# chalharu/rust-compression

Measured on AMD Instinct MI355X. Metric: BZip2 level-9 encode MB/s (input bytes, HBM-resident in and out: the kernels' rate; value_end_to_end is host buffer to host buffer at the C ABI), higher is better.
Workload: dtype u8/u32

## Files before the change

### rust-compression_amd/csrc/k_bwt.hip

```cpp
#include "bzgpu.h"
#include <algorithm>
#include <atomic>
#include <cstdio>
#include <cstdlib>
#include <vector>

namespace bzgpu {
constexpr u32 kGhSpan = 8;
constexpr u32 kSymSpan = 8;

enum { SRC_TEXT = 0, SRC_PAIRS = 1, SRC_MM = 2, SRC_WALK = 3, SRC_SURV = 4, SRC_LISTG = 5,
       SRC_TEXTK = 6, SRC_WALKK = 7, SRC_MMK = 8,
       SRC_MMC = 9,
       SRC_PERJ = 10,
       SRC_PACKED = 11,
       SRC_PERJK = 12 };
template <int SRC> struct src_is_list {
    static constexpr bool value = (SRC == SRC_PAIRS || SRC == SRC_SURV || SRC == SRC_LISTG || SRC == SRC_PERJ || SRC == SRC_PERJK || SRC == SRC_PACKED);
};

struct KeyInfo {
    u8 bits;
    u8 chars;
    u8 pad[2];
};

__device__ __forceinline__ u32 pkey(const u8 *__restrict__ pt, u32 j, u32 bits, u32 chars)
{
    const u32 bitpos = j * bits, kb = bits * chars;
    u64 v;
    __builtin_memcpy(&v, pt + (bitpos >> 3), 8);
    v = __builtin_bswap64(v);
    return (u32)(v >> (64u - (bitpos & 7u) - kb)) & (u32)((1ull << kb) - 1ull);
}

__device__ __forceinline__ u64 newbits_lane_word(const u64 *__restrict__ bits, size_t base, u32 wbase, u32 cnt, u32 l, bool fill)
{
    const u32 rowbase = wbase + l * 64u;
    u64 m = 0;
    if (l < 17u && rowbase < cnt) m = bits[(base + rowbase) >> 6];
    if (fill && l < 17u) {
        if (rowbase >= cnt) m = ~0ull;
        else if (cnt - rowbase < 64u) m |= ~0ull << (cnt - rowbase);
    }
    return m;
}

constexpr u32 kPerWords = kSlot / 64u;
constexpr u32 kPerSetBytes = 2u * kPerWords * 8u + ((kPerWords + 1u) * 4u + 7u) / 8u * 8u;
static_assert((size_t)kPerK * kPerSetBytes <= (size_t)kTilesPerBlock * 3 * kMaxBins * 4, "the period tables do not fit the digit-count slot");
__host__ __device__ __forceinline__ bool per_in_counts(const BwtArgs &a) { return a.gh_tiles != nullptr; }
__host__ __device__ __forceinline__ u32 per_kmax(const BwtArgs &a) { return per_in_counts(a) ? kPerK : (kSlot / kPerSetBytes < kPerK ? kSlot / kPerSetBytes : kPerK); }
__device__ __forceinline__ const u8 *per_set(const BwtArgs &a, u32 lb, u32 i)
{
    const u8 *base = per_in_counts(a) ? reinterpret_cast<const u8 *>(a.gh_tiles + (size_t)lb * kTilesPerBlock * 3 * kMaxBins)
                                      : a.flags + (size_t)lb * kSlot;
    return base + (size_t)i * kPerSetBytes;
}
__device__ __forceinline__ const u64 *per_mis(const BwtArgs &a, u32 lb, u32 i) { return reinterpret_cast<const u64 *>(per_set(a, lb, i)); }
__device__ __forceinline__ const u64 *per_lt(const BwtArgs &a, u32 lb, u32 i) { return per_mis(a, lb, i) + kPerWords; }
__device__ __forceinline__ const u32 *per_nxt(const BwtArgs &a, u32 lb, u32 i) { return reinterpret_cast<const u32 *>(per_mis(a, lb, i) + 2u * kPerWords); }
__device__ __forceinline__ u32 per_first_mis(const BwtArgs &a, u32 lb, u32 i, u32 x)
{
    const u32 w = x >> 6;
    const u64 here = per_mis(a, lb, i)[w] & (~0ull << (x & 63u));
    return here ? (w << 6) + (u32)__builtin_ctzll(here) : per_nxt(a, lb, i)[w + 1u];
}
__device__ __forceinline__ bool per_lt_at(const BwtArgs &a, u32 lb, u32 i, u32 n, u32 m)
{
    if (m >= n) m -= n;
    return (per_lt(a, lb, i)[m >> 6] >> (m & 63u)) & 1ull;
}
__device__ __forceinline__ bool per_key_ascending(const BwtArgs &a, u32 lb, u32 n, u32 depth, u32 j)
{
    const u32 kmax = per_kmax(a);
    for (u32 i = 0; i < kmax; ++i) {
        const u32 p = a.lin_p[(size_t)lb * kPerK + i];
        if (p == 0u) break;
        if (j + p < n) {
            const u32 m = per_first_mis(a, lb, i, j);
            if (m - j >= depth) return per_lt_at(a, lb, i, n, m);
        }
        if (j >= p) {
            const u32 m = per_first_mis(a, lb, i, j - p);
            if (m - (j - p) >= depth) return per_lt_at(a, lb, i, n, m);
        }
    }
    return true;
}

__device__ __forceinline__ bool per_ekey(const BwtArgs &a, u32 lb, const u8 *__restrict__ text, u32 n, u32 depth, u32 x, u32 &key)
{
    const u32 kmax = per_kmax(a);
    for (u32 i = 0; i < kmax; ++i) {
        const u32 p = a.lin_p[(size_t)lb * kPerK + i];
        if (p == 0u) break;
        if (p > depth) continue;
        const u32 m = per_first_mis(a, lb, i, x);
        const u32 e = m - x + p;
        if (e < depth) continue;
        u32 mp = (m >= n ? m - n : m) + p;
        mp = mp >= n ? mp - n : mp;
        const bool up = per_lt_at(a, lb, i, n, m);
        const u32 ec = e < 0xFFFFFu ? e : 0xFFFFFu;
        key = up ? ((1u << 28) | ((0xFFFFFu - ec) << 8) | (u32)text[mp]) : ((ec << 8) | (u32)text[mp]);
        return true;
    }
    return false;
}

constexpr u32 kLinkMax = 8;
__device__ __forceinline__ u8 *group_bytes(const BwtArgs &a, u32 lb)
{
    return a.per_aux + (size_t)lb * kMtfStride * 2u;
}

// ... 913 lines not shown
    const u32 gshift = 20u + kbits;
    const bool haveB = posB < len;
    u64 eA[16], eB[16];
    loc_fill(eA, s_e, posA, len, l, le_mask, gshift, gcarryA);
    if (haveB) loc_fill(eB, s_e, posB, len, l, le_mask, gshift, gcarryB);
    const u32 gbits = groups > 1u ? 32u - (u32)__builtin_clz(groups - 1u) : 0u;
    const u32 npass = (kbits + gbits + kLocBits - 1u) / kLocBits;
    u32 *cntA = s_cnt[w], *cntB = s_cnt[kLocWaves + w];
    u16 *cnt16 = reinterpret_cast<u16 *>(&s_cnt[0][0]);
#pragma unroll 1
    for (u32 p = 0; p < npass; ++p) {
        const u32 shift = 20u + p * kLocBits;
        u32 rnkA[16], rnkB[16];
        loc_rank(eA, rnkA, cntA, posA, len, l, shift);
        if (haveB) loc_rank(eB, rnkB, cntB, posB, len, l, shift);
        else {
#pragma unroll
            for (u32 q = 0; q < kLocBins / 2 / 64; ++q) cntB[q * 64u + l] = 0;
        }
        __syncthreads();
        u32 tot;
        {
            const u32 dg = threadIdx.x;
            u32 run = 0;
#pragma unroll
            for (u32 k = 0; k < kLocSets; ++k) {
                const u32 c = cnt16[k * kLocBins + dg];
                cnt16[k * kLocBins + dg] = (u16)run;
                run += c;
            }
            tot = run;
        }
        const u32 inc = wave_incl_sum(tot);
        if (l == 63) s_wsum[w] = inc;
        __syncthreads();
        {
            u32 carry = 0;
            for (u32 k = 0; k < w; ++k) carry += s_wsum[k];
            s_tpre[threadIdx.x] = (u16)(carry + inc - tot);
        }
        __syncthreads();
        loc_move(eA, rnkA, cntA, s_tpre, s_e, posA, len, l, shift);
        if (haveB) loc_move(eB, rnkB, cntB, s_tpre, s_e, posB, len, l, shift);
        __syncthreads();
        if (p + 1 < npass) {
            loc_reload(eA, s_e, posA, len, l);
            if (haveB) loc_reload(eB, s_e, posB, len, l);
        }
    }
    {
        bool bad = false;
        for (u32 i = threadIdx.x; i < len; i += kLocThreads) {
            const u64 x = s_e[i];
            if (i && (s_e[i - 1] >> 20) > (x >> 20)) bad = true;
            const u32 v = (u32)x & 0xFFFFFu;
            Vout[base + s0 + i] = v;
            Kout[base + s0 + i] = Rb[v] & ~kFinalBit;
        }
        if (__ballot(bad) && l == 0) s_bad = 1u;
    }
    __syncthreads();
    if (threadIdx.x == 0 && s_bad) atomicAdd(&a.loc_stats[LOC_STAT_SURV_FAIL], 1u);
}

template <bool INIT>
__global__ __launch_bounds__(kSortThreads) void k_group_flags(BwtArgs a, u32 step, const u32 *__restrict__ K,
                                                               const u32 *__restrict__ V,
                                                               const u8 *__restrict__ impure = nullptr)
{
    __shared__ int s_old, s_new;
    u32 tile, lb;
    xcd_remap(gridDim.x, a.nb, tile, lb);
    if (lb == 0xFFFFFFFFu) return;
    const BlockDesc d = a.blocks[lb];
    const u32 n = d.n;
    const u32 cnt = a.count[lb];
    const u32 start = tile * kSortTile;
    if (start >= cnt) return;
    const KeyInfo ki = reinterpret_cast<const KeyInfo *>(a.keyinfo)[lb];
    const u32 hm = INIT ? (u32)ki.chars % n : (((u32)ki.chars * 2u) << step) % n;
    const u8 *text = a.rle + d.rle_off;
    const u8 *pt = a.ptext + (size_t)lb * kSlot;
    const size_t base = (size_t)lb * kSlot;
    if (INIT && a.pb_gate[lb] == 0u) K = a.KA;
    if (threadIdx.x == 0) {
        s_old = -1;
        s_new = -1;
    }
    __syncthreads();
    const u32 w = threadIdx.x >> 6, l = threadIdx.x & 63u;
    int last_old = -1, last_new = -1;
    const u32 first = start + w * 1024u + l;
    u32 g[16], s1[16], s2[16];
    u32 pg0 = 0, ps10 = 0, ps20 = 0;
    {
        u32 jj[16];
#pragma unroll
        for (u32 r = 0; r < 16; ++r) {
            const u32 idx = first + r * 64u;
            const u32 c = idx < cnt ? idx : cnt - 1u;
            const u32 kk = ld_stream(K + base + c);
            const u32 t = ld_stream(V + base + c) + hm;
            jj[r] = t >= n ? t - n : t;
            g[r] = INIT ? 0u : kk;
            s1[r] = kk;
            s2[r] = 0;
        }
        u32 pj = 0;
        const bool need_prev = (l == 0) && (first > 0) && (first < cnt);
        if (need_prev) {
            const u32 kk = K[base + first - 1];
            pg0 = INIT ? 0u : kk;
            ps10 = kk;
            const u32 t = V[base + first - 1] + hm;
            pj = t >= n ? t - n : t;
        }
        if (INIT) {
#pragma unroll
            for (u32 r = 0; r < 16; ++r) s2[r] = pkey(pt, jj[r], ki.bits, ki.chars);
            if (need_prev) ps20 = pkey(pt, pj, ki.bits, ki.chars);
        } else if (impure) {
            const bool per = a.lin_p[(size_t)lb * kPerK] != 0u;
            const u64 d64 = ((u64)ki.chars * 2u) << step;
            const u32 depth = d64 < n ? (u32)d64 : n;
#pragma unroll
            for (u32 r = 0; r < 16; ++r) {
                const u32 jr = jj[r] >= hm ? jj[r] - hm : jj[r] + n - hm;
                const u32 im = impure[base + g[r]];
                u32 ek;
                s1[r] = (im == 2u || (per && im == 0u)) ? jr + 1u : ((per && a.per_wide && per_ekey(a, lb, text, n, depth, jr, ek)) ? ek + 1u : 0u);
            }
            if (need_prev) {
                const u32 jr = pj >= hm ? pj - hm : pj + n - hm;
                const u32 im = impure[base + pg0];
                u32 ek;
                ps10 = (im == 2u || (per && im == 0u)) ? jr + 1u : ((per && a.per_wide && per_ekey(a, lb, text, n, depth, jr, ek)) ? ek + 1u : 0u);
            }
        } else {
#pragma unroll
            for (u32 r = 0; r < 16; ++r) s1[r] = a.R[base + jj[r]];
            if (need_prev) ps10 = a.R[base + pj];
        }
    }
#pragma unroll
    for (u32 r = 0; r < 16; ++r) {
        const u32 idx = first + r * 64u;
        const bool ok = idx < cnt;
        u32 pg = wave_shr1(g[r]), p1 = wave_shr1(s1[r]), p2 = wave_shr1(s2[r]);
        const u32 qg = (r == 0) ? pg0 : wave_lane(g[(r + 15) & 15], 63);
        const u32 q1 = (r == 0) ? ps10 : wave_lane(s1[(r + 15) & 15], 63);
        const u32 q2 = (r == 0) ? ps20 : wave_lane(s2[(r + 15) & 15], 63);
        if (l == 0) {
            pg = qg;
            p1 = q1;
            p2 = q2;
        }
        bool ns = false;
        if (ok) {
            const bool os = (idx == 0) || (g[r] != pg);
            ns = os || (s1[r] != p1) || (s2[r] != p2);
            a.flags[base + idx] = (u8)((os ? 1u : 0u) | (ns ? 2u : 0u));
            if (os) last_old = (int)idx;
            if (ns) last_new = (int)idx;
        }
        const u64 mrow = __ballot(ns);
        if (l == 0 && idx < cnt) a.newbits[(base + idx) >> 6] = mrow;
    }
// ... 166 lines not shown
        const u32 mine = c0 + c1;
        const u32 inc = wave_incl_sum(mine);
        if (l == 63) s_wsum[w] = inc;
        u32 g0 = 0, g1 = 0;
        u32 *cur = a.bin_cursor + (size_t)lb * 1024u;
        if (c0) g0 = atomicAdd(&cur[b0], c0);
        if (c1) g1 = atomicAdd(&cur[b0 + 1], c1);
        __syncthreads();
        u32 carry = 0;
        for (u32 k = 0; k < w; ++k) carry += s_wsum[k];
        const u32 ex = carry + inc - mine;
        s_bpre[b0] = (u16)ex;
        s_bpre[b0 + 1] = (u16)(ex + c0);
        s_bcnt[b0] = (b0 << kRankBinShift) + g0;
        s_bcnt[b0 + 1] = ((b0 + 1u) << kRankBinShift) + g1;
    }
    __syncthreads();
#pragma unroll
    for (u32 r = 0; r < 16; ++r) {
        if (lrank[r] != 0xFFFFFFFFu) {
            const u32 bin = jv[r] >> kRankBinShift;
            const u32 pos = (u32)s_bpre[bin] + lrank[r];
            s_stage[pos] = word[r];
            s_binof[pos] = (u16)bin;
        }
    }
    __syncthreads();
    const u32 total = (cnt - start) < kSortTile ? (cnt - start) : kSortTile;
#pragma unroll
    for (u32 k = 0; k < 16; ++k) {
        const u32 i = k * kSortThreads + threadIdx.x;
        if (i < total) {
            const u32 bin = s_binof[i];
            W[base + s_bcnt[bin] + (i - (u32)s_bpre[bin])] = s_stage[i];
        }
    }
}

constexpr u32 kLbNone = 0xFFFFFu;
#ifdef BZ_REFINE_TIMING
#define RF_T(k) do { __syncthreads(); const u64 t_ = __builtin_readcyclecounter(); if (threadIdx.x == 0) atomicAdd(&a.loc_stats[16 + (INIT ? 8 : 0) + (k)], (u32)((t_ - t_prev) >> 4)); t_prev = t_; } while (0)
#else
#define RF_T(k) do { } while (0)
#endif
template <bool INIT>
__global__ __launch_bounds__(kSortThreads, 4) void k_group_refine(BwtArgs a, u32 step, u32 next_step, u32 round,
                                                                const u32 *__restrict__ K,
                                                                const u32 *__restrict__ V, u32 *__restrict__ W,
                                                                u32 epoch)
{
    constexpr u32 NW = kSortThreads / 64;
    __shared__ int s_carry_old, s_carry_new;
    __shared__ int s_wold[NW], s_wnew[NW];
    __shared__ u32 s_nonfinal, s_ticket;
    __shared__ u32 s_stage[kSortTile];
    __shared__ u16 s_binof[kSortTile];
    __shared__ u16 s_bpre[1024];
    __shared__ u16 s_bdst[1024];
    __shared__ u32 s_wsum[NW];
    u32 (*s_gh)[1024] = reinterpret_cast<u32 (*)[1024]>(s_stage);
    u32 *s_bcnt = s_stage + 2048;
#ifdef BZ_REFINE_TIMING
    u64 t_prev = __builtin_readcyclecounter();
#endif
    const u32 xcd = (u32)__builtin_amdgcn_s_getreg(20 | (3 << 11)) & 7u;
    const u32 my_tiles = a.tiles * ((a.nb + 7u - xcd) / 8u);
    if (threadIdx.x == 0) s_ticket = atomicAdd(&a.tickets[(size_t)epoch * 8u + xcd], 1u);
    __syncthreads();
    const u32 slot = s_ticket;
    if (slot >= my_tiles) return;
    const u32 b8 = slot / a.tiles;
    const u32 tile = slot - b8 * a.tiles;
    const u32 lb = b8 * 8u + xcd;
    const BlockDesc d = a.blocks[lb];
    const u32 n = d.n;
    const u8 *__restrict__ text = a.rle + d.rle_off;
    const u32 cnt = a.count[lb];
    const u32 start = tile * kSortTile;
    if (start >= cnt) return;
    const KeyInfo ki = reinterpret_cast<const KeyInfo *>(a.keyinfo)[lb];
    const u32 hm = INIT ? (u32)ki.chars % n : (((u32)ki.chars * 2u) << step) % n;
    const u8 *pt = a.ptext + (size_t)lb * kSlot;
    const size_t base = (size_t)lb * kSlot;
    if (INIT && a.pb_gate[lb] == 0u) K = a.KA;
    for (u32 i = threadIdx.x; i < 3072u; i += kSortThreads) s_stage[i] = 0;
    if (threadIdx.x == 0) s_nonfinal = 0;
    const u32 w = threadIdx.x >> 6, l = threadIdx.x & 63u;
    const u32 wbase = start + w * 1024u;
    const u32 first = wbase + l;

    RF_T(0);
    u32 gk[16], jv[16], s1[16], s2[16];
    u32 pg0 = 0, ps10 = 0, ps20 = 0;
    u32 ng0 = 0, ns10 = 0, ns20 = 0;
    const bool need_prev = (l == 0) && (first > 0) && (first < cnt);
    const bool need_next = (l == 63) && (wbase + 1024u < cnt);
    {
#pragma unroll
        for (u32 r = 0; r < 16; ++r) {
            const u32 idx = first + r * 64u;
            const u32 c = idx < cnt ? idx : cnt - 1u;
            const u32 kk = ld_stream(K + base + c);
            const u32 vv = ld_stream(V + base + c);
            if (INIT) {
                jv[r] = vv;
                const u32 t = vv + hm;
                s2[r] = t >= n ? t - n : t;
                gk[r] = 0u;
                s1[r] = kk;
            } else {
                jv[r] = vv & 0xFFFFFu;
                gk[r] = kk & 0xFFFFFu;
                s1[r] = (kk >> 20) | ((vv >> 20) << 12);
                s2[r] = 0u;
            }
        }
        u32 pj = 0, nj = 0;
        if (need_prev) {
            const u32 kk = K[base + wbase - 1], vv = V[base + wbase - 1];
            pg0 = INIT ? 0u : (kk & 0xFFFFFu);
            ps10 = INIT ? kk : ((kk >> 20) | ((vv >> 20) << 12));
            const u32 t = vv + hm;
            pj = t >= n ? t - n : t;
        }
        if (need_next) {
            const u32 kk = K[base + wbase + 1024u], vv = V[base + wbase + 1024u];
            ng0 = INIT ? 0u : (kk & 0xFFFFFu);
            ns10 = INIT ? kk : ((kk >> 20) | ((vv >> 20) << 12));
            const u32 t = vv + hm;
            nj = t >= n ? t - n : t;
        }
        if (INIT) {
#pragma unroll
            for (u32 r = 0; r < 16; ++r) s2[r] = pkey(pt, s2[r], ki.bits, ki.chars);
            if (need_prev) ps20 = pkey(pt, pj, ki.bits, ki.chars);
            if (need_next) ns20 = pkey(pt, nj, ki.bits, ki.chars);
        }
    }
    RF_T(1);
    u64 mo[16] = {}, mn[16];
    int wl_old = -1, wl_new = -1;
#pragma unroll
    for (u32 r = 0; r < 16; ++r) {
        const u32 idx = first + r * 64u;
        const bool ok = idx < cnt;
        u32 pg = wave_shr1(gk[r]), p1 = wave_shr1(s1[r]), p2 = wave_shr1(s2[r]);
        const u32 qg = (r == 0) ? pg0 : wave_lane(gk[(r + 15) & 15], 63);
        const u32 q1 = (r == 0) ? ps10 : wave_lane(s1[(r + 15) & 15], 63);
        const u32 q2 = (r == 0) ? ps20 : wave_lane(s2[(r + 15) & 15], 63);
        if (l == 0) {
            pg = qg;
            p1 = q1;
            p2 = q2;
        }
        const bool os = ok && ((idx == 0) || (!INIT && gk[r] != pg));
        const bool ns = ok && (os || (s1[r] != p1) || (s2[r] != p2));
        mn[r] = __ballot(ns);
        if (l == 0 && ok) a.newbits[(base + idx) >> 6] = mn[r];
        if (mn[r]) wl_new = (int)(wbase + r * 64u + 63u - __clzll(mn[r]));
        if (!INIT) {
            mo[r] = __ballot(os);
            if (mo[r]) wl_old = (int)(wbase + r * 64u + 63u - __clzll(mo[r]));
        }
    }
    bool next_after = true;
    if (need_next) next_after = (gk[15] != ng0) || (s1[15] != ns10) || (s2[15] != ns20);
    next_after = wave_lane((u32)next_after, 63) != 0u;
    if (l == 0) {
        s_wold[w] = INIT ? 0 : wl_old;
        s_wnew[w] = wl_new;
    }
    u32 finbits = 0;
    u32 lcol[16];
#pragma unroll
    for (u32 r = 0; r < 16; ++r) {
        const u32 idx = first + r * 64u;
        bool next_new;
        if (idx + 1 >= cnt) next_new = true;
        else if (l < 63) next_new = (mn[r] >> (l + 1)) & 1ull;
        else if (r < 15) next_new = mn[(r + 1) & 15] & 1ull;
        else next_new = next_after;
        const bool fin = (idx < cnt) && ((mn[r] >> l) & 1ull) && next_new;
        finbits |= (fin ? 1u : 0u) << r;
        lcol[r] = 0;
        if (INIT && fin) lcol[r] = text[jv[r] ? jv[r] - 1u : n - 1u];
    }
    __syncthreads();
    RF_T(2);
    if (threadIdx.x == 0) {
        int lo = INIT ? 0 : -1, ln = -1;
        for (u32 k = 0; k < NW; ++k) {
            lo = s_wold[k] > lo ? s_wold[k] : lo;
            ln = s_wnew[k] > ln ? s_wnew[k] : ln;
        }
        u32 *mystate = a.tile_state + ((size_t)lb * kTilesPerBlock + tile) * kMaxBins;
        const u32 etag = epoch << 22;
        const u32 f0 = etag | (tile ? kLbAgg : kLbIncl);
        const u32 vo = lo >= 0 ? (u32)lo : kLbNone, vn = ln >= 0 ? (u32)ln : kLbNone;
        st_sc1_x4(mystate, make_uint4(f0 | vo, f0 | vn, f0, f0));
        int co = -1, cn = -1;
        if (tile) {
            u32 spins = 0;
            for (u32 p = tile; p > 0 && (co < 0 || cn < 0);) {
                --p;
                const u32 *src = a.tile_state + ((size_t)lb * kTilesPerBlock + p) * kMaxBins;
                uint4 v = ld_sc1_x4(src);
                while ((v.x >> 22) != epoch || (v.x & kLbFlagMask) == 0u || (v.y >> 22) != epoch || (v.y & kLbFlagMask) == 0u) {
                    if (lb_give_up(spins, a.sort_err, kLbSpinMax >> 3)) {
                        atomicExch(a.sort_err, 1u);
                        v = make_uint4(etag | kLbIncl, etag | kLbIncl, 0, 0);
                        break;
                    }
                    __builtin_amdgcn_s_sleep(2);
                    v = ld_sc1_x4(src);
                }
                const u32 xo = v.x & kLbValMask, xn = v.y & kLbValMask;
                if (co < 0 && xo != kLbNone) co = (int)xo;
                if (cn < 0 && xn != kLbNone) cn = (int)xn;
            }
// ... 1167 lines not shown
        bytes[i] = 0;
        seconds[i] = 0;
    }
}

template <int SRC, int BITS>
static void radix_pass(hipStream_t st, const BwtArgs &a, u32 shift, u32 h, const u32 *Kin, const u32 *Vin,
                       u32 *Kout, u32 *Vout, u64 elems, KernelProf *prof, u32 *Ktmp = nullptr, u32 tiles = kTilesPerBlock)
{
    const dim3 grid(tiles, xcd_grid_y(a.nb));
    const u64 rd_hist = (SRC == SRC_TEXT) ? 1 : (SRC == SRC_PAIRS ? 4 : (SRC == SRC_WALK ? 5 : 8));
    const u64 rd_scat = (SRC == SRC_TEXT) ? 1 : (SRC == SRC_WALK ? 5 : 8);
    int p = prof ? prof->begin(st, KID_RADIX_HIST, elems * rd_hist) : -1;
    hipLaunchKernelGGL((k_radix_hist<SRC, BITS>), grid, dim3(kSortThreads), 0, st, a, shift, h, Kin, Vin, Ktmp);
    if (prof) prof->end(st, p);
    p = prof ? prof->begin(st, KID_RADIX_SCAN, (u64)a.nb * kTilesPerBlock * (1u << BITS) * 8u) : -1;
    hipLaunchKernelGGL((k_radix_scan<SRC, BITS>), dim3(a.nb), dim3(kSortThreads), 0, st, a);
    if (prof) prof->end(st, p);
    p = prof ? prof->begin(st, KID_RADIX_SCATTER, elems * (rd_scat + 8)) : -1;
    if (SRC == SRC_TEXT && Ktmp)
        hipLaunchKernelGGL((k_radix_scatter<SRC_TEXTK, BITS>), grid, dim3(kSortThreads), 0, st, a, shift, h, Ktmp,
                           Vin, Kout, Vout);
    else if (SRC == SRC_WALK && Ktmp)
        hipLaunchKernelGGL((k_radix_scatter<SRC_WALKK, BITS>), grid, dim3(kSortThreads), 0, st, a, shift, h, Ktmp,
                           Vin, Kout, Vout);
    else if (SRC == SRC_MM && Ktmp)
        hipLaunchKernelGGL((k_radix_scatter<SRC_MMK, BITS>), grid, dim3(kSortThreads), 0, st, a, shift, h, Ktmp,
                           Vin, Kout, Vout);
    else if (SRC == SRC_PERJ && Ktmp)
        hipLaunchKernelGGL((k_radix_scatter<SRC_PERJK, BITS>), grid, dim3(kSortThreads), 0, st, a, shift, h, Ktmp,
                           Vin, Kout, Vout);
    else if ((SRC == SRC_SURV || SRC == SRC_LISTG) && Ktmp)
        hipLaunchKernelGGL((k_radix_scatter<SRC_PAIRS, BITS>), grid, dim3(kSortThreads), 0, st, a, shift, h, Ktmp,
                           Vin, Kout, Vout);
    else
        hipLaunchKernelGGL((k_radix_scatter<SRC, BITS>), grid, dim3(kSortThreads), 0, st, a, shift, h, Kin, Vin,
                           Kout, Vout);
    if (prof) prof->end(st, p);
}

static u32 next_epoch(hipStream_t st, const BwtArgs &a)
{
    u32 e = *a.epoch + 1u;
    if (e >= kSortEpochs) {
        (void)hipMemsetAsync(a.tile_state_all, 0, a.tile_state_bytes, st);
        (void)hipMemsetAsync(a.tickets, 0, (size_t)kSortEpochs * 8 * 4, st);
        e = 1;
    }
    *a.epoch = e;
    return e;
}

template <int SRC, int BITS, bool WRITE_K = true, bool PACK_OUT = false>
static void fused_pass(hipStream_t st, const BwtArgs &a, u32 shift, u32 h, const u32 *Kin, const u32 *Vin, u32 *Kout,
                       u32 *Vout, u32 dpos, u64 elems, KernelProf *prof, u64 out_elems = ~0ull,
                       const u32 *gate = nullptr)
{
    const dim3 grid(a.tiles, xcd_grid_y(a.nb));
    const u64 rd = (SRC == SRC_TEXTK || SRC == SRC_PACKED) ? 4 : ((SRC == SRC_TEXT) ? 1 : ((SRC == SRC_WALK) ? 5 : (SRC == SRC_MMC ? 9 : 8)));
    const u32 e = next_epoch(st, a);
    if (out_elems == ~0ull) out_elems = elems;
    const int p = prof ? prof->begin(st, KID_RADIX_SCATTER_LB, elems * rd + out_elems * ((WRITE_K && !PACK_OUT) ? 8 : 4)) : -1;
    hipLaunchKernelGGL((k_radix_scatter_lb<SRC, BITS, WRITE_K, PACK_OUT>), grid, dim3(kSortTile / 16), 0, st, a, shift, h, Kin, Vin, Kout, Vout, dpos, e, gate);
    if (prof) prof->end(st, p);
}

static bool fused_pass_ok(hipStream_t st, const BwtArgs &a, u32 epoch)
{
    static const bool fail_test = getenv("BZ_ONESWEEP_FAILTEST") != nullptr;
    if (fail_test) return false;
    u32 tk[8], gave_up = 0;
    {
        const MailSeg sg[2] = {{tk, a.tickets + (size_t)epoch * 8u, sizeof(tk)}, {&gave_up, a.sort_err, 4}};
        if (mail_fetch(st, sg, 2) != 0) return false;
    }
    if (gave_up) return false;
    const u32 want = a.tiles * (xcd_grid_y(a.nb) / 8u);
    for (u32 x = 0; x < 8; ++x)
        if (tk[x] != want) return false;
    return true;
}

template <int B0, int B1, int B2>
static bool init_sort_fused(hipStream_t st, const BwtArgs &a, u64 total_n, KernelProf *prof)
{
    const dim3 grid(a.tiles, xcd_grid_y(a.nb));
    int p = prof ? prof->begin(st, KID_GHIST_TEXT, total_n * 1) : -1;
    hipLaunchKernelGGL((k_ghist_text<B0, B1, B2>), dim3((a.tiles + kGhSpan - 1u) / kGhSpan, xcd_grid_y(a.nb)), dim3(kSortThreads), 0, st, a, (u32 *)nullptr);
    if (prof) prof->end(st, p);
    p = prof ? prof->begin(st, KID_GHIST_SCAN, (u64)a.nb * kTilesPerBlock * 3 * 1024 * 4 / kGhSpan) : -1;
    hipLaunchKernelGGL(k_ghist_scan, dim3(a.nb), dim3(kSortThreads), 0, st, a, 3u, 1u << B0, 1u << B1, 1u << B2, 0u, kGhSpan);
    if (prof) prof->end(st, p);
    static const bool stale_tickets_test = getenv("BZ_TEST_STALE_TICKETS") && atoi(getenv("BZ_TEST_STALE_TICKETS")) != 0;
    if (stale_tickets_test && *a.epoch + 1u < kSortEpochs)
        (void)hipMemsetD32Async((hipDeviceptr_t)(a.tickets + (size_t)(*a.epoch + 1u) * 8u),
                                (int)(a.tiles * (xcd_grid_y(a.nb) / 8u)), 8, st);
    fused_pass<SRC_TEXT, B0>(st, a, 0, 0, nullptr, nullptr, a.KA, a.VA, 0, total_n, prof);
    if (!fused_pass_ok(st, a, *a.epoch)) return false;
    fused_pass<SRC_PAIRS, B1, true, true>(st, a, B0, 0, a.KA, a.VA, nullptr, a.VB, 1, total_n, prof);
    (void)hipMemsetAsync(a.pb_gate, 1, a.nb * sizeof(u32), st);
    fused_pass<SRC_PACKED, B2, false>(st, a, 20, 0, nullptr, a.VB, nullptr, a.VA, 2, total_n, prof);
    const u32 *gate = nullptr;
    fused_pass<SRC_WALK, B0>(st, a, 0, 0, a.KA, a.VA, a.KB, a.VB, 0, total_n, prof, ~0ull, gate);
    fused_pass<SRC_PAIRS, B1>(st, a, B0, 0, a.KB, a.VB, a.KA, a.VA, 1, total_n, prof, ~0ull, gate);
    fused_pass<SRC_PAIRS, B2>(st, a, B0 + B1, 0, a.KA, a.VA, a.KB, a.SA, 2, total_n, prof, ~0ull, gate);
    return true;
}

void launch_block_symbols(hipStream_t st, const BwtArgs &a, u32 *inuse_bits, u8 *sym_code, u8 *keyinfo)
{
    const dim3 grid(kTilesPerBlock, xcd_grid_y(a.nb));
    (void)hipMemsetAsync(inuse_bits, 0, (size_t)a.nb * 8 * sizeof(u32), st);
    hipLaunchKernelGGL(k_block_symbols, dim3((a.tiles + kSymSpan - 1u) / kSymSpan, xcd_grid_y(a.nb)), dim3(kSortThreads), 0, st, a, inuse_bits);
    hipLaunchKernelGGL(k_key_params, dim3(a.nb), dim3(256), 0, st, inuse_bits, sym_code, keyinfo);
    hipLaunchKernelGGL(k_pack_text, grid, dim3(kSortThreads), 0, st, a, a.ptext);
}

template <int B0, int B1, int B2>
static void init_sort(hipStream_t st, const BwtArgs &a, u64 total_n, KernelProf *prof)
{
    radix_pass<SRC_TEXT, B0>(st, a, 0, 0, nullptr, nullptr, a.KA, a.VA, total_n, prof, a.KB);
    radix_pass<SRC_PAIRS, B1>(st, a, B0, 0, a.KA, a.VA, a.KB, a.VB, total_n, prof);
    radix_pass<SRC_PAIRS, B2>(st, a, B0 + B1, 0, a.KB, a.VB, a.KA, a.VA, total_n, prof);
    radix_pass<SRC_WALK, B0>(st, a, 0, 0, a.KA, a.VA, a.KB, a.VB, total_n, prof, a.KA);
    radix_pass<SRC_PAIRS, B1>(st, a, B0, 0, a.KB, a.VB, a.KA, a.VA, total_n, prof);
    radix_pass<SRC_PAIRS, B2>(st, a, B0 + B1, 0, a.KA, a.VA, a.KB, a.SA, total_n, prof);
}


static int run_bwt_once(hipStream_t st, const BwtArgs &a_in, u32 max_n, u64 total_n, unsigned long long *h_active,
                        u64 *sorted_elems, KernelProf *prof, u64 *round_active, bool wide_keys, u32 min_chars,
                        bool allow_fused)
{
    BwtArgs a = a_in;
    if (!allow_fused || a.fused_state[0]) a.fused = 0;
    a.tiles = std::min<u32>(kTilesPerBlock, std::max<u32>(1u, (max_n + kSortTile - 1u) / kSortTile));
    const dim3 grid(a.tiles, xcd_grid_y(a.nb));
    (void)hipMemsetAsync(a.active, 0, 64 * sizeof(unsigned long long), st);
    (void)hipMemsetAsync(a.maxnf, 0, 64 * sizeof(u32), st);
    (void)hipMemsetAsync(a.nonfinal, 0, a.nb * sizeof(u32), st);
    if (a.sort_err) (void)hipMemsetAsync(a.sort_err, 0, 4, st);

    bool fused = a.fused != 0;
    const u32 epoch_first = *a.epoch + 1u;
    if (fused) {
        const bool ok = wide_keys ? init_sort_fused<11, 11, 10>(st, a, total_n, prof) : init_sort_fused<10, 10, 10>(st, a, total_n, prof);
        if (!ok) {
            fprintf(stderr, "bz2_mi355x: fused radix passes disabled (tile tickets / look-back check failed)\n");
            a.fused_state[0] = 1;
            a.fused_state[1] += 1;
            fused = false;
            a.fused = 0;
            (void)hipMemsetAsync(a.sort_err, 0, 4, st);
        }
    }
    if (!fused) {
        (void)hipMemsetAsync(a.pb_gate, 1, a.nb * sizeof(u32), st);
        if (wide_keys) init_sort<11, 11, 10>(st, a, total_n, prof);
        else init_sort<10, 10, 10>(st, a, total_n, prof);
    }
    static const bool want_refine = !(getenv("BZ_FUSED_REFINE") && atoi(getenv("BZ_FUSED_REFINE")) == 0);
    const bool refine = fused && want_refine;
    int p;
    (void)hipMemsetAsync(a.bin_cursor, 0, (size_t)a.nb * 1024 * sizeof(u32), st);
    if (refine) {
        const u32 e = next_epoch(st, a);
        p = prof ? prof->begin(st, KID_GROUP_REFINE, total_n * 14) : -1;
        hipLaunchKernelGGL((k_group_refine<true>), grid, dim3(kSortThreads), 0, st, a, 0u, 0u, 0u, a.KB, a.SA, a.KA, e);
        if (prof) prof->end(st, p);
    } else {
        p = prof ? prof->begin(st, KID_GROUP_FLAGS, total_n * 9) : -1;
        hipLaunchKernelGGL((k_group_flags<true>), grid, dim3(kSortThreads), 0, st, a, 0u, a.KB, a.SA);
        if (prof) prof->end(st, p);
        p = prof ? prof->begin(st, KID_GROUP_APPLY, total_n * 13) : -1;
        hipLaunchKernelGGL((k_group_apply<true>), grid, dim3(kSortThreads), 0, st, a, 0u, 0u, a.KB, a.SA, a.KA);
        if (prof) prof->end(st, p);
    }
    p = prof ? prof->begin(st, KID_RANK_PLACE, total_n * 8) : -1;
    hipLaunchKernelGGL(k_rank_place, grid, dim3(kSortThreads), 0, st, a, a.KA);
    if (prof) prof->end(st, p);

    u32 *cK = a.KB, *cV = a.VB;
    u32 *fK = a.KA, *fV = a.VA;
    const u32 *lastV = a.SA;
    u32 step = 0;
    int rounds = 0;
    u32 slot = 0;
    bool period_done = false;
    bool last_doubled = false, links_pay = true;
    u64 link_m = 0;
    if (!(a.gh_tiles && a.per_aux)) a.per_links = 0;
    const u32 links_on = a.per_links;
    bool surv_local_ok = true;
    u32 list_tiles = a.tiles;
    while (true) {
        {
            const MailSeg sg[2] = {{h_active, a.active + slot, sizeof(unsigned long long)}, {h_active + 1, a.maxnf + slot, sizeof(u32)}};
            if (mail_fetch(st, sg, 2) != 0) return -1;
        }
        const u64 m = *h_active;
        const u32 list_tiles_prev = list_tiles;
        const u32 mx = *reinterpret_cast<const u32 *>(h_active + 1);
        {
            list_tiles = (mx + kSortTile - 1) / kSortTile + 1u;
            if (list_tiles > kTilesPerBlock) list_tiles = kTilesPerBlock;
        }
        const dim3 grid_list(list_tiles, xcd_grid_y(a.nb)), grid_prev(list_tiles_prev, xcd_grid_y(a.nb));
        if (sorted_elems) *sorted_elems += m;
        if (round_active && slot < 64) round_active[slot] += m;
        if (m == 0 || step > 24 || ((u64)(2u * min_chars) << step) >= max_n) break;
        ++slot;
        ++rounds;
        bool carried = false;
        u32 trace_worst = 0;
        static const bool bwt_trace = getenv("BZ_BWT_TRACE") != nullptr;
        if (bwt_trace) {
            std::vector<u32> nf(a.nb);
            (void)hipMemcpyAsync(nf.data(), a.nonfinal, a.nb * 4, hipMemcpyDeviceToHost, st);
            (void)hipStreamSynchronize(st);
            trace_worst = (u32)(std::max_element(nf.begin(), nf.end()) - nf.begin());
        }
        (void)hipMemsetAsync(a.nonfinal, 0, a.nb * sizeof(u32), st);
        static const int want_period = [] {
            const char *e = getenv("BZ_PERIOD_ROUND");
            return !e ? 1 : (e[0] == 'b' ? 2 : (atoi(e) != 0 ? 1 : 0));
        }();
        const bool deep = want_period == 2 ? (rounds >= 3 && m * 4 >= total_n * 3)
                                           : ((rounds >= 2 && ((u64)mx * 4 >= (u64)max_n * 3 || m * 4 >= total_n * 3)) ||
                                              (rounds == 1 && m * 64 >= total_n * 63));
        const bool per_round = want_period != 0 && !period_done && deep;
        if (link_m) {
            if ((link_m - m) * 4 < link_m) links_pay = false;
            link_m = 0;
        }
        const bool link_round = !per_round && links_on && period_done && last_doubled && links_pay && m * 256 >= total_n;
        constexpr u64 surv_num = 1, surv_den = 4;
        if (bwt_trace)
            fprintf(stderr, "bz2_mi355x: sort round %d (h = %llu): %llu of %llu rotations unordered, at most %u in one block (block %u; of %u)%s\n",
                    rounds, (unsigned long long)(2u * min_chars) << step, (unsigned long long)m, (unsigned long long)total_n, mx,
                    trace_worst, max_n, per_round ? ": period round" : (link_round ? ": link round" : (m * surv_den < total_n * surv_num ? ": survivor form" : ": walk form")));
        u8 *impure = a.ptext;
        last_doubled = !(per_round || link_round);
        if (per_round || link_round) {
            if (per_round) period_done = true;
            else link_m = m;
            (void)hipMemsetAsync(impure, 0, (size_t)a.nb * kSlot, st);
            const bool links = links_on != 0 && !(per_round && rounds == 1);
            a.per_links = links ? 1u : 0u;
            u32 *midx = cK;
            if (links) (void)hipMemsetAsync(midx, 0, (size_t)a.nb * kSlot * sizeof(u32), st);
            hipLaunchKernelGGL(k_survivor_compact, grid_prev, dim3(kSortThreads), 0, st, a, lastV, fV, links ? midx : nullptr, per_round ? 1u : 0u);
// ... 215 lines not shown
```

Before: 13580.

## Recompute init keys from packed text in refine, skipping key output from last radix passes

In the fused init sort, when refine is enabled the last two radix passes stop writing key arrays and use the value-only/packed variants. k_group_refine<true> then recomputes both key halves (s1, s2) directly from the packed text with a new pkey2 helper that reads 12 bytes once. This removes K reads in refine and K writes in the radix passes, at the cost of extra bit-extraction work and a dependence on the packed-text path staying consistent with the radix key layout. The pb_gate K redirection is also dropped from the group kernels.

```diff
diff --git a/rust-compression_amd/csrc/k_bwt.hip b/rust-compression_amd/csrc/k_bwt.hip
--- a/rust-compression_amd/csrc/k_bwt.hip
+++ b/rust-compression_amd/csrc/k_bwt.hip
@@ -32,6 +32,19 @@
     __builtin_memcpy(&v, pt + (bitpos >> 3), 8);
     v = __builtin_bswap64(v);
     return (u32)(v >> (64u - (bitpos & 7u) - kb)) & (u32)((1ull << kb) - 1ull);
+}
+
+__device__ __forceinline__ void pkey2(const u8 *__restrict__ pt, u32 j, u32 bits, u32 chars, u32 &k1, u32 &k2)
+{
+    const u32 bitpos = j * bits, kb = bits * chars, o = bitpos & 7u;
+    u32 w[3];
+    __builtin_memcpy(w, pt + (bitpos >> 3), 12);
+    const u64 hi = __builtin_bswap64((u64)w[0] | ((u64)w[1] << 32));
+    const u64 lo = (u64)__builtin_bswap32(w[2]) << 32;
+    const u32 mask = (u32)((1ull << kb) - 1ull);
+    const u32 t = o + kb;
+    k1 = (u32)(hi >> (64u - t)) & mask;
+    k2 = (u32)(((hi << t) | (lo >> (64u - t))) >> (64u - kb)) & mask;
 }
 
 __device__ __forceinline__ u64 newbits_lane_word(const u64 *__restrict__ bits, size_t base, u32 wbase, u32 cnt, u32 l, bool fill)
@@ -1111,7 +1124,6 @@
     const u8 *text = a.rle + d.rle_off;
     const u8 *pt = a.ptext + (size_t)lb * kSlot;
     const size_t base = (size_t)lb * kSlot;
-    if (INIT && a.pb_gate[lb] == 0u) K = a.KA;
     if (threadIdx.x == 0) {
         s_old = -1;
         s_new = -1;
@@ -1444,7 +1456,6 @@
     const u32 hm = INIT ? (u32)ki.chars % n : (((u32)ki.chars * 2u) << step) % n;
     const u8 *pt = a.ptext + (size_t)lb * kSlot;
     const size_t base = (size_t)lb * kSlot;
-    if (INIT && a.pb_gate[lb] == 0u) K = a.KA;
     for (u32 i = threadIdx.x; i < 3072u; i += kSortThreads) s_stage[i] = 0;
     if (threadIdx.x == 0) s_nonfinal = 0;
     const u32 w = threadIdx.x >> 6, l = threadIdx.x & 63u;
@@ -1462,41 +1473,41 @@
         for (u32 r = 0; r < 16; ++r) {
             const u32 idx = first + r * 64u;
             const u32 c = idx < cnt ? idx : cnt - 1u;
-            const u32 kk = ld_stream(K + base + c);
             const u32 vv = ld_stream(V + base + c);
             if (INIT) {
                 jv[r] = vv;
-                const u32 t = vv + hm;
-                s2[r] = t >= n ? t - n : t;
                 gk[r] = 0u;
-                s1[r] = kk;
+                pkey2(pt, vv, ki.bits, ki.chars, s1[r], s2[r]);
             } else {
+                const u32 kk = ld_stream(K + base + c);
                 jv[r] = vv & 0xFFFFFu;
                 gk[r] = kk & 0xFFFFFu;
                 s1[r] = (kk >> 20) | ((vv >> 20) << 12);
                 s2[r] = 0u;
             }
         }
-        u32 pj = 0, nj = 0;
+        u32 pv = 0, nv = 0;
         if (need_prev) {
-            const u32 kk = K[base + wbase - 1], vv = V[base + wbase - 1];
-            pg0 = INIT ? 0u : (kk & 0xFFFFFu);
-            ps10 = INIT ? kk : ((kk >> 20) | ((vv >> 20) << 12));
-            const u32 t = vv + hm;
-            pj = t >= n ? t - n : t;
+            const u32 vv = V[base + wbase - 1];
+            if (!INIT) {
+                const u32 kk = K[base + wbase - 1];
+                pg0 = kk & 0xFFFFFu;
+                ps10 = (kk >> 20) | ((vv >> 20) << 12);
+            }
+            pv = vv;
         }
         if (need_next) {
-            const u32 kk = K[base + wbase + 1024u], vv = V[base + wbase + 1024u];
-            ng0 = INIT ? 0u : (kk & 0xFFFFFu);
-            ns10 = INIT ? kk : ((kk >> 20) | ((vv >> 20) << 12));
-            const u32 t = vv + hm;
-            nj = t >= n ? t - n : t;
+            const u32 vv = V[base + wbase + 1024u];
+            if (!INIT) {
+                const u32 kk = K[base + wbase + 1024u];
+                ng0 = kk & 0xFFFFFu;
+                ns10 = (kk >> 20) | ((vv >> 20) << 12);
+            }
+            nv = vv;
         }
         if (INIT) {
-#pragma unroll
-            for (u32 r = 0; r < 16; ++r) s2[r] = pkey(pt, s2[r], ki.bits, ki.chars);
-            if (need_prev) ps20 = pkey(pt, pj, ki.bits, ki.chars);
-            if (need_next) ns20 = pkey(pt, nj, ki.bits, ki.chars);
+            if (need_prev) pkey2(pt, pv, ki.bits, ki.chars, ps10, ps20);
+            if (need_next) pkey2(pt, nv, ki.bits, ki.chars, ns10, ns20);
         }
     }
     RF_T(1);
@@ -2830,7 +2841,7 @@
 }
 
 template <int B0, int B1, int B2>
-static bool init_sort_fused(hipStream_t st, const BwtArgs &a, u64 total_n, KernelProf *prof)
+static bool init_sort_fused(hipStream_t st, const BwtArgs &a, u64 total_n, KernelProf *prof, bool keys_out)
 {
     const dim3 grid(a.tiles, xcd_grid_y(a.nb));
     int p = prof ? prof->begin(st, KID_GHIST_TEXT, total_n * 1) : -1;
@@ -2850,8 +2861,13 @@
     fused_pass<SRC_PACKED, B2, false>(st, a, 20, 0, nullptr, a.VB, nullptr, a.VA, 2, total_n, prof);
     const u32 *gate = nullptr;
     fused_pass<SRC_WALK, B0>(st, a, 0, 0, a.KA, a.VA, a.KB, a.VB, 0, total_n, prof, ~0ull, gate);
-    fused_pass<SRC_PAIRS, B1>(st, a, B0, 0, a.KB, a.VB, a.KA, a.VA, 1, total_n, prof, ~0ull, gate);
-    fused_pass<SRC_PAIRS, B2>(st, a, B0 + B1, 0, a.KA, a.VA, a.KB, a.SA, 2, total_n, prof, ~0ull, gate);
+    if (keys_out) {
+        fused_pass<SRC_PAIRS, B1>(st, a, B0, 0, a.KB, a.VB, a.KA, a.VA, 1, total_n, prof, ~0ull, gate);
+        fused_pass<SRC_PAIRS, B2>(st, a, B0 + B1, 0, a.KA, a.VA, a.KB, a.SA, 2, total_n, prof, ~0ull, gate);
+    } else {
+        fused_pass<SRC_PAIRS, B1, true, true>(st, a, B0, 0, a.KB, a.VB, nullptr, a.VA, 1, total_n, prof, ~0ull, gate);
+        fused_pass<SRC_PACKED, B2, false>(st, a, 20, 0, nullptr, a.VA, nullptr, a.SA, 2, total_n, prof, ~0ull, gate);
+    }
     return true;
 }
 
@@ -2891,8 +2907,10 @@
 
     bool fused = a.fused != 0;
     const u32 epoch_first = *a.epoch + 1u;
+    static const bool want_refine = !(getenv("BZ_FUSED_REFINE") && atoi(getenv("BZ_FUSED_REFINE")) == 0);
     if (fused) {
-        const bool ok = wide_keys ? init_sort_fused<11, 11, 10>(st, a, total_n, prof) : init_sort_fused<10, 10, 10>(st, a, total_n, prof);
+        const bool keys_out = !want_refine;
+        const bool ok = wide_keys ? init_sort_fused<11, 11, 10>(st, a, total_n, prof, keys_out) : init_sort_fused<10, 10, 10>(st, a, total_n, prof, keys_out);
         if (!ok) {
             fprintf(stderr, "bz2_mi355x: fused radix passes disabled (tile tickets / look-back check failed)\n");
             a.fused_state[0] = 1;
@@ -2907,14 +2925,13 @@
         if (wide_keys) init_sort<11, 11, 10>(st, a, total_n, prof);
         else init_sort<10, 10, 10>(st, a, total_n, prof);
     }
-    static const bool want_refine = !(getenv("BZ_FUSED_REFINE") && atoi(getenv("BZ_FUSED_REFINE")) == 0);
     const bool refine = fused && want_refine;
     int p;
     (void)hipMemsetAsync(a.bin_cursor, 0, (size_t)a.nb * 1024 * sizeof(u32), st);
     if (refine) {
         const u32 e = next_epoch(st, a);
-        p = prof ? prof->begin(st, KID_GROUP_REFINE, total_n * 14) : -1;
-        hipLaunchKernelGGL((k_group_refine<true>), grid, dim3(kSortThreads), 0, st, a, 0u, 0u, 0u, a.KB, a.SA, a.KA, e);
+        p = prof ? prof->begin(st, KID_GROUP_REFINE, total_n * 10) : -1;
+        hipLaunchKernelGGL((k_group_refine<true>), grid, dim3(kSortThreads), 0, st, a, 0u, 0u, 0u, (const u32 *)nullptr, a.SA, a.KA, e);
         if (prof) prof->end(st, p);
     } else {
         p = prof ? prof->begin(st, KID_GROUP_FLAGS, total_n * 9) : -1;
```

Result: faster. 13800 (median of 6 runs) (+1.6%).
